# fishmarch/MS-SLAM

Measured on AMD Instinct MI355X. Metric: Mkeypoints/s extract+describe, KITTI-00-like stereo 1241x376, 2000 feat/frame, higher is better.
Workload: dtype u8

## Files before the change

### ms-slam_amd/csrc/gauss7_stream_device.h

```cpp
#pragma once
#include <hip/hip_runtime.h>
#include <stdint.h>

#include "orb_device.h"

namespace msorb {

typedef unsigned short ushort2v __attribute__((ext_vector_type(2)));

constexpr int kGaussRows = 28;
struct GaussTaps { uint32_t k[7]; };

struct BlurPlan {
    int block_begin[kMaxLevels + 1];
    int bx_count[kMaxLevels];
    int nlevels;
    uint32_t bx_magic[kMaxLevels];
    uint32_t image_magic;
};

__device__ __forceinline__ int refl101(int p, int len) { return p < 0 ? -p : (p >= len ? 2 * (len - 1) - p : p); }

constexpr int kGaussLanesOut = 62;
template <int ROWS, bool EDGE>
__device__ __forceinline__ void gauss7_strip(const uint8_t* __restrict__ sb, uint8_t* __restrict__ db, int src_pitch, int dst_pitch,
                                             int h, int y0, uint32_t xl, int x0, bool store, uint32_t sel_w1, uint32_t sel_w2a,
                                             uint32_t sel_w2b) {
    static_assert(ROWS % 28 == 0, "strips start on a multiple of 4 rows and the row loop is unrolled over 4 x 7 rows");
    uint8_t* const dblk = db + blur_tile_off((uint32_t)max(x0, 0), 0u, (uint32_t)dst_pitch);
    uint32_t blk[4] = {0u, 0u, 0u, 0u};
    auto load_row = [&](int r) {
        int yy = refl101(y0 - 3 + r, h);
        yy = min(max(yy, 0), h - 1);
        return *reinterpret_cast<const uint32_t*>(sb + (uint32_t)yy * (uint32_t)src_pitch + xl);
    };
    constexpr uint32_t k0 = 18, k1 = 34, k2 = 48, k3 = 56;
    constexpr uint32_t A0 = (k0 << 8) | (k1 << 16) | (k2 << 24), B0 = k3 | (k2 << 8) | (k1 << 16) | (k0 << 24);
    constexpr uint32_t A1 = (k0 << 16) | (k1 << 24), B1 = k2 | (k3 << 8) | (k2 << 16) | (k1 << 24), C1 = k0;
    constexpr uint32_t A2 = (k0 << 24), B2 = k1 | (k2 << 8) | (k3 << 16) | (k2 << 24), C2 = k1 | (k0 << 8);
    constexpr uint32_t B3 = k0 | (k1 << 8) | (k2 << 16) | (k3 << 24), C3 = k2 | (k1 << 8) | (k0 << 16);
    auto row_sums = [&](uint32_t w1, uint32_t hs[4]) {
        uint32_t w0 = (uint32_t)__builtin_amdgcn_update_dpp(0, (int)w1, 0x138 , 0xf, 0xf, true);
        uint32_t w2 = (uint32_t)__builtin_amdgcn_update_dpp(0, (int)w1, 0x130 , 0xf, 0xf, true);
        if (EDGE) {
            if (x0 == 0) w0 = __builtin_amdgcn_perm(0u, w1, 0x01020300u);
            const uint32_t n2 = __builtin_amdgcn_perm(w1, w0, sel_w2a) | __builtin_amdgcn_perm(0u, w2, sel_w2b);
            w1 = __builtin_amdgcn_perm(w1, w0, sel_w1);
            w2 = n2;
        }
        hs[0] = __builtin_amdgcn_udot4(w1, B0, __builtin_amdgcn_udot4(w0, A0, 0u, false), false);
        hs[1] = __builtin_amdgcn_udot4(w2, C1, __builtin_amdgcn_udot4(w1, B1, __builtin_amdgcn_udot4(w0, A1, 0u, false), false), false);
        hs[2] = __builtin_amdgcn_udot4(w2, C2, __builtin_amdgcn_udot4(w1, B2, __builtin_amdgcn_udot4(w0, A2, 0u, false), false), false);
        hs[3] = __builtin_amdgcn_udot4(w2, C3, __builtin_amdgcn_udot4(w1, B3, 0u, false), false);
    };
    const ushort2v K01 = {(unsigned short)k0, (unsigned short)k1}, K23 = {(unsigned short)k2, (unsigned short)k3},
                   K45 = {(unsigned short)k2, (unsigned short)k1};
    uint32_t acc[7][4];
    uint32_t hs[4], hp[4] = {0, 0, 0, 0};
    uint32_t warm[6], nxt[7];
#pragma unroll
    for (int r = 0; r < 6; r++) warm[r] = load_row(r);
#pragma unroll
    for (int u = 0; u < 7; u++) nxt[u] = load_row(6 + u);
#pragma unroll
    for (int r = 0; r < 6; r++) {
        row_sums(warm[r], hs);
#pragma unroll
        for (int j = 0; j < 4; j++) {
            if (r >= 1) {
                const ushort2v P = __builtin_bit_cast(ushort2v, hp[j] | (hs[j] << 16));
                acc[(r - 1) % 7][j] = __builtin_amdgcn_udot2(P, K01, 32768u, false);
                if (r >= 3) acc[(r - 3) % 7][j] = __builtin_amdgcn_udot2(P, K23, acc[(r - 3) % 7][j], false);
                if (r >= 5) acc[(r - 5) % 7][j] = __builtin_amdgcn_udot2(P, K45, acc[(r - 5) % 7][j], false);
            }
            hp[j] = hs[j];
        }
    }
#pragma unroll
    for (int it = 0; it < ROWS / 7; it++) {
        if (y0 + 7 * it >= h) break;
        uint32_t cur[7];
#pragma unroll
        for (int u = 0; u < 7; u++) cur[u] = nxt[u];
        if (it + 1 < ROWS / 7) {
#pragma unroll
            for (int u = 0; u < 7; u++) nxt[u] = load_row(6 + 7 * (it + 1) + u);
        }
#pragma unroll
        for (int u = 0; u < 7; u++) {
            const int r = 6 + 7 * it + u;
            row_sums(cur[u], hs);
            uint32_t q[4];
#pragma unroll
            for (int j = 0; j < 4; j++) {
                const ushort2v P = __builtin_bit_cast(ushort2v, hp[j] | (hs[j] << 16));
                q[j] = __umul24(hs[j], k0) + acc[u % 7][j];
                acc[(5 + u) % 7][j] = __builtin_amdgcn_udot2(P, K01, 32768u, false);
                acc[(3 + u) % 7][j] = __builtin_amdgcn_udot2(P, K23, acc[(3 + u) % 7][j], false);
                acc[(1 + u) % 7][j] = __builtin_amdgcn_udot2(P, K45, acc[(1 + u) % 7][j], false);
                hp[j] = hs[j];
            }
            const int o = r - 6;
            if (y0 + o < h) {
                const uint32_t packed = __builtin_amdgcn_perm(__builtin_amdgcn_perm(q[3], q[2], 0x0c0c0602u),
                                                              __builtin_amdgcn_perm(q[1], q[0], 0x0c0c0602u), 0x05040100u);
                blk[o & 3] = packed;
                if ((o & 3) == 3 || y0 + o == h - 1) {
                    if (store) *reinterpret_cast<uint4*>(dblk + (uint32_t)((y0 + o) >> 2) * ((uint32_t)dst_pitch * 4u)) = make_uint4(blk[0], blk[1], blk[2], blk[3]);
                }
            }
        }
    }
}

template <int ROWS>
__device__ __forceinline__ void gauss7_stream_body(const PyramidView& src, const PyramidView& dst, const BlurPlan& plan, const int tile, const int wave_in_block) {
    const int blocks_per_image = plan.block_begin[plan.nlevels];
    const int img = plan.image_magic ? (int)__umulhi((uint32_t)tile, plan.image_magic) : tile / blocks_per_image, blk = tile - img * blocks_per_image;
    int level = 0;
    while (level + 1 < plan.nlevels && blk >= plan.block_begin[level + 1]) level++;
    const int rem = blk - plan.block_begin[level];
    const int by = plan.bx_magic[level] ? (int)__umulhi((uint32_t)rem, plan.bx_magic[level]) : rem / plan.bx_count[level];
    const int bx = rem - by * plan.bx_count[level];
    const LevelView sv = src.lv[level], dv = dst.lv[level];
    const int lane = threadIdx.x & 63;
    const int x0 = (bx * kGaussLanesOut + lane - 1) * 4;
    const int y0 = (by * 4 + __builtin_amdgcn_readfirstlane(wave_in_block)) * ROWS;
    if (y0 >= sv.h) return;
    const bool store = lane >= 1 && (lane <= kGaussLanesOut || x0 + 4 >= sv.w) && x0 < sv.w;
    const bool border_block = (bx + 1) * kGaussLanesOut * 4 + 7 > sv.w;
    uint32_t sel_w1 = 0x07060504u, sel_w2a = 0x0c0c0c0cu, sel_w2b = 0x03020100u;
    if (border_block && x0 + 7 > sv.w && x0 < sv.w) {
        sel_w1 = 0; sel_w2a = 0; sel_w2b = 0;
        for (int b = 0; b < 8; b++) {
            const int x = x0 + b;
            int idx = b + 4;
            if (x >= sv.w) idx = max(2 * (sv.w - 1) - x, x0 - 4) - x0 + 4;
            if (b < 4) sel_w1 |= (uint32_t)idx << (8 * b);
            else {
                sel_w2a |= (uint32_t)(idx < 8 ? idx : 0x0c) << (8 * (b - 4));
                sel_w2b |= (uint32_t)(idx >= 8 ? idx - 8 : 0x0c) << (8 * (b - 4));
            }
        }
    }
    const uint32_t xl = (uint32_t)min(max(x0, 0), sv.pitch - 4);
    const uint8_t* sb = sv.base + (size_t)img * sv.img_stride;
    uint8_t* db = const_cast<uint8_t*>(dv.base) + (size_t)img * dv.img_stride;
    if (border_block || bx == 0)
        gauss7_strip<ROWS, true>(sb, db, sv.pitch, dv.pitch, sv.h, y0, xl, x0, store, sel_w1, sel_w2a, sel_w2b);
    else
        gauss7_strip<ROWS, false>(sb, db, sv.pitch, dv.pitch, sv.h, y0, xl, x0, store, sel_w1, sel_w2a, sel_w2b);
}

struct FrameBlurJob {
    PyramidView src, dst;
    BlurPlan plan;
    int blocks = 0;
};
bool make_frame_blur_job(const PyramidView& src, const PyramidView& dst, int n_images, const Semantics& sem, FrameBlurJob* job);

}
```

### ms-slam_amd/csrc/orb_kernels.hip

```cpp
#include <hip/hip_runtime.h>

#include <algorithm>
#include <string>
#include <stdint.h>
#include <stdlib.h>

#include "lds_limit.h"
#include "orb_device.h"
#include "gauss7_stream_device.h"
#include "sincosf_restated.h"

namespace msorb {

__global__ __launch_bounds__(256) void pyr_resize_kernel(LevelView src, LevelView dst, uint8_t* __restrict__ dst_base,
                                                         const ResizeTap* __restrict__ tx,
                                                         const ResizeTap* __restrict__ ty, int single_stage) {
    const int img = blockIdx.z;
    const int dy = blockIdx.y * 4 + (threadIdx.x >> 6);
    const int dx0 = (blockIdx.x * 64 + (threadIdx.x & 63)) * 4;
    if (dy >= dst.h || dx0 >= dst.w) return;
    const ResizeTap vy = ty[dy];
    const uint8_t* s0 = src.base + (size_t)img * src.img_stride + (size_t)vy.i0 * src.pitch;
    const uint8_t* s1 = src.base + (size_t)img * src.img_stride + (size_t)vy.i1 * src.pitch;
    const int b0 = vy.c0, b1 = vy.c1;
// ... 356 lines not shown
        colp_off = tr.colp;
        baseA = tr.rows_tbase >> 16;
    } else {
        int g_own, y_b;
        if (!by_wave) {
            const int strip = (int)(__umul24((uint32_t)tid, magic) >> 20);
            g_own = tid - strip * G;
            y_b = strip * R;
        } else {
            const int sl = (int)(__umul24((uint32_t)lane, magic) >> 20);
            g_own = lane - sl * G;
            const int y_w = (int)(((T == 128 ? cd.yw128 : cd.yw256) >> sw) & 255u);
            y_b = sl < (int)cd.spw ? y_w + sl * R : dh;
        }
        nrows = min(max(dh - y_b, 0), R);
        const int c_own = c_lo + 4 * g_own;
        const int xg = ga + c_own;
        const int vlo = min(max(x_lo - xg, 0), 4), vhi = min(max(x_hi - xg, 0), 4);
        Hm = (0x80808080u << (8 * vlo)) & (uint32_t)(0x0080808080ull >> (8 * (4 - vhi)));
        if (vlo >= 4) Hm = 0;
        colp_off = __umul24((uint32_t)y_b, P) + (uint32_t)c_own;
        baseA = (uint32_t)(((y_b + 3) << 7) | c_own);
    }
    tbase[tid] = (uint16_t)baseA;
    auto quick_test = [&](int th, uint32_t& wA, uint32_t& wB) {
        wA = 0; wB = 0;
        const uint8_t* colp = &tile[colp_off];
        uint32_t cw[GEO::kMaxR + 6], lw[GEO::kMaxR], rw_[GEO::kMaxR];
#pragma unroll
        for (int r = 0; r < GEO::kMaxR + 6; r++)
            if (r < 9 || r - 6 < R) cw[r] = *reinterpret_cast<const uint32_t*>(colp + r * P);
#pragma unroll
        for (int k = 0; k < GEO::kMaxR; k++)
            if (k < 3 || k < R) {
                lw[k] = *reinterpret_cast<const uint32_t*>(colp + (k + 3) * P - 4);
                rw_[k] = *reinterpret_cast<const uint32_t*>(colp + (k + 3) * P + 4);
            }
        const ushort2v t2 = __builtin_bit_cast(ushort2v, (uint32_t)th * 0x00010001u);
#pragma unroll
        for (int k = 0; k < GEO::kMaxR; k++) {
            if (k >= 3 && k >= R) break;
            const uint32_t V = cw[k + 3], U = cw[k], D = cw[k + 6];
            const uint32_t R3 = __builtin_amdgcn_alignbyte(rw_[k], V, 3);
            const uint32_t L3 = __builtin_amdgcn_alignbyte(V, lw[k], 1);
            const uint32_t Ve = V & 0x00ff00ffu, Vo = (V >> 8) & 0x00ff00ffu;
            const uint32_t Ae = __builtin_bit_cast(uint32_t, __builtin_elementwise_sub_sat(__builtin_bit_cast(ushort2v, Ve), t2));
            const uint32_t Ao = __builtin_bit_cast(uint32_t, __builtin_elementwise_sub_sat(__builtin_bit_cast(ushort2v, Vo), t2));
            const uint32_t Qd = ~(Ae | (Ao << 8));
            const uint32_t Be = __builtin_bit_cast(uint32_t, __builtin_elementwise_sub_sat(__builtin_bit_cast(ushort2v, Ve ^ 0x00ff00ffu), t2));
            const uint32_t Bo = __builtin_bit_cast(uint32_t, __builtin_elementwise_sub_sat(__builtin_bit_cast(ushort2v, Vo ^ 0x00ff00ffu), t2));
            const uint32_t Qb = Be | (Bo << 8);
            const uint32_t one = 0x01010101u;
            const uint32_t X = (__builtin_amdgcn_lerp(U, Qd, one) & __builtin_amdgcn_lerp(D, Qd, one)) |
                               (__builtin_amdgcn_lerp(L3, Qd, one) & __builtin_amdgcn_lerp(R3, Qd, one));
            const uint32_t Y = (__builtin_amdgcn_lerp(U, Qb, 0u) | __builtin_amdgcn_lerp(D, Qb, 0u)) &
                               (__builtin_amdgcn_lerp(L3, Qb, 0u) | __builtin_amdgcn_lerp(R3, Qb, 0u));
            const uint32_t hm = k < nrows ? Hm : 0u;
            const uint32_t z = (Y & hm) | ((~X & hm) >> 1);
            if (k < 4) wA |= z >> (6 - 2 * k);
            else wB |= z >> (6 - 2 * (k - 4));
        }
    };
    __syncthreads();

    const int sc_off = 4 - c_lo;
    Cand16* const out = slots + (size_t)img * slots_per_image + cd.slot_off;
    int n_emitted = 0;
    for (int pass = 0; pass < 2; pass++) {
        const int th = pass ? min_th : ini_th;
        uint32_t wA, wB;
        quick_test(th, wA, wB);
        const int cnt = __popc(wA) + __popc(wB);
        int n_work = 0;
        const int my_base = block_excl_scan<T / 64>(cnt, lane, wave, wave_tot[0], &n_work);

        const uint32_t baseB = baseA + (4u << 7);
        int w_begin = 0, n_corner = 0;
        if (n_work <= GEO::kWorkCap) {
            uint16_t* wp = &work[my_base];
            const uint32_t idA = (uint32_t)tid << 5, idB = idA | (1u << (5 + (T == 128 ? 7 : 8)));
            for (uint32_t w = wA; w; w &= w - 1) *wp++ = (uint16_t)(idA | (uint32_t)__builtin_ctz(w));
            for (uint32_t w = wB; w; w &= w - 1) *wp++ = (uint16_t)(idB | (uint32_t)__builtin_ctz(w));
            __syncthreads();
            w_begin = wave * ((((n_work + T / 64 - 1) / (T / 64)) + 63) & ~63);
            const int w_end = min(w_begin + ((((n_work + T / 64 - 1) / (T / 64)) + 63) & ~63), n_work);
            n_corner = 0;
            for (int i0 = w_begin; i0 < w_end; i0 += 64) {
                const int i = i0 + lane;
                bool corner = false;
                int ce = 0;
                if (i < w_end) {
                    const int id = work[i];
                    const int e = tbase[(id >> 5) & (T - 1)] + lut[id & 31] + ((id >> (5 + (T == 128 ? 7 : 8))) << 9);
                    const int ty = (e >> 7) & 127, tx = e & 127;
                    const int A = fast_arc_contrast_pk<GEO>(&tile[(int)__umul24((uint32_t)ty, P) + tx], (e & 0x8000) ? -1 : 1);
                    if (A > th) {
                        score[(int)__umul24((uint32_t)(ty - 2), SP) + tx + sc_off] = (uint8_t)(A - 1);
                        ce = e & 0x3FFF;
                        corner = true;
                    }
                }
                const unsigned long long bm = __ballot(corner);
                if (corner)
                    work[w_begin + n_corner + (int)__builtin_amdgcn_mbcnt_hi((uint32_t)(bm >> 32), __builtin_amdgcn_mbcnt_lo((uint32_t)bm, 0u))] = (uint16_t)ce;
                n_corner += __popcll(bm);
            }
        } else {
#pragma unroll 1
            for (int half = 0; half < 2; half++)
#pragma unroll 1
                for (uint32_t w = half ? wB : wA; w; w &= w - 1) {
                    const int e = lut[__builtin_ctz(w)] + (half ? baseB : baseA);
                    const int ty = (e >> 7) & 127, tx = e & 127;
                    const int A = fast_arc_contrast_pk<GEO>(&tile[(int)__umul24((uint32_t)ty, P) + tx], (e & 0x8000) ? -1 : 1);
                    if (A > th) score[(int)__umul24((uint32_t)(ty - 2), SP) + tx + sc_off] = (uint8_t)(A - 1);
                }
        }
        __syncthreads();

        if (n_work <= GEO::kWorkCap) {
            constexpr int wpr = GEO::kWordsPerRow;
            const int nwords = dh * wpr;
            uint32_t mine_keep = 0;
            {
                int slot = 0;
                for (int m0 = 0; m0 < n_corner; m0 += 64, slot++) {
                    if (m0 + lane >= n_corner) continue;
                    const int e = work[w_begin + m0 + lane];
                    const int ty = e >> 7, tx = e & 127;
                    const uint8_t* q = &score[(int)__umul24((uint32_t)(ty - 2), SP) + tx + sc_off];
                    const int sv = q[0];
                    int m = max3i(q[-SP - 1], q[-SP], q[-SP + 1]);
                    m = max3i(m, q[-1], q[1]);
                    m = max(m, max3i(q[SP - 1], q[SP], q[SP + 1]));
                    if (sv > m) {
                        const int bx = tx - c_lo, by = ty - 3;
                        const int b = by * (32 * wpr) + bx;
                        atomicOr(&kbits[b >> 5], 1u << (b & 31));
                        mine_keep |= 1u << slot;
                    }
                }
            }
            __syncthreads();
            const uint32_t myword = tid < nwords ? kbits[tid] : 0u;
            int n_out = 0;
            const int wprefix = block_excl_scan<T / 64>(__popc(myword), lane, wave, wave_tot[1], &n_out);
            if (tid < nwords) kprefix[tid] = wprefix;
            __syncthreads();
            {
                int slot = 0;
                for (int m0 = 0; m0 < n_corner; m0 += 64, slot++) {
                    if (!(mine_keep & (1u << slot))) continue;
                    const int e = work[w_begin + m0 + lane];
                    const int ty = e >> 7, tx = e & 127;
                    const int b = (ty - 3) * (32 * wpr) + (tx - c_lo);
                    const int rank = kprefix[b >> 5] + __popc(kbits[b >> 5] & ((1u << (b & 31)) - 1u));
                    Cand16 c;
                    c.x = (uint16_t)(ga + tx - kMinBorder);
                    c.y = (uint16_t)(cd.y0 + ty - kMinBorder);
                    c.score = score[(int)__umul24((uint32_t)(ty - 2), SP) + tx + sc_off];
                    c.pad = 0;
                    out[rank] = c;
                }
            }
            n_emitted = n_out;
        } else {
            const int n_task = dh * G;
            uint32_t tid_here = (uint32_t)tid;
            asm volatile("" : "+v"(tid_here));
            const int t_begin = (int)(__umul24(tid_here, (uint32_t)n_task) / T),
                      t_end = (int)(__umul24(tid_here + 1u, (uint32_t)n_task) / T);
            uint64_t keep = 0;
            {
                int y = (int)(__umul24((uint32_t)t_begin, magic) >> 20);
                int g = t_begin - y * G;
                for (int task = t_begin, k = 0; task < t_end; task++, k++) {
                    const uint8_t* sp = &score[(y + 1) * SP + 4 + 4 * g];
                    const uint32_t S = *reinterpret_cast<const uint32_t*>(sp);
                    if (S) {
#pragma unroll
                        for (int j = 0; j < 4; j++) {
                            const int sv = (S >> (8 * j)) & 255;
                            if (sv) {
                                const uint8_t* q = sp + j;
                                int m = max3i(q[-SP - 1], q[-SP], q[-SP + 1]);
                                m = max3i(m, q[-1], q[1]);
                                m = max(m, max3i(q[SP - 1], q[SP], q[SP + 1]));
                                if (sv > m) keep |= 1ull << (4 * k + j);
                            }
                        }
                    }
                    if (++g == G) { g = 0; y++; }
                }
            }
            int n_out = 0;
            int pos = block_excl_scan<T / 64>(__popcll(keep), lane, wave, wave_tot[1], &n_out);
            if (keep) {
                int y = (int)(__umul24((uint32_t)t_begin, magic) >> 20);
                int g = t_begin - y * G;
                uint64_t m = keep;
                for (int task = t_begin; task < t_end; task++, m >>= 4) {
                    uint32_t m4 = (uint32_t)m & 15u;
                    while (m4) {
                        const int j = __ffs(m4) - 1;
                        m4 &= m4 - 1;
                        Cand16 c;
                        c.x = (uint16_t)(gx0 + 4 * g + j - kMinBorder);
                        c.y = (uint16_t)(cd.y0 + 3 + y - kMinBorder);
                        c.score = score[(y + 1) * SP + 4 + 4 * g + j];
                        c.pad = 0;
                        out[pos++] = c;
                    }
                    if (++g == G) { g = 0; y++; }
                }
            }
            n_emitted = n_out;
        }
        if (n_emitted > 0 || pass == 1 || ini_th == min_th) break;
        __syncthreads();
        clear_planes();
        __syncthreads();
    }
    if (tid == 0) cell_count[(size_t)img * n_cells + cell_id] = n_emitted;
}

template <bool ALIGNED, class GEO>
__global__ __launch_bounds__(GEO::kThreads, GEO::kMinWaves) void fast_cells_kernel(PyramidView pyr, const CellDesc* __restrict__ cells,
                                                         const FastThreadRec* __restrict__ ttab,
                                                         int ini_th, int min_th, int slots_per_image,
                                                         Cand16* __restrict__ slots, int* __restrict__ cell_count,
                                                         int n_cells, uint32_t gx_magic) {
    fast_cells_body<ALIGNED, GEO>(pyr, cells, ttab, ini_th, min_th, slots_per_image, slots, cell_count, n_cells, gx_magic,
                                  blockIdx.y * gridDim.x + blockIdx.x, gridDim.x, gridDim.x * gridDim.y);
}

__global__ __launch_bounds__(256) void cand_scan_cells_kernel(const int* __restrict__ cell_count, int n_cells,
// ... 346 lines not shown
    return a;
}

__device__ __forceinline__ int wave_sum_dpp(int v) {
    v += __builtin_amdgcn_update_dpp(0, v, 0xB1 , 0xf, 0xf, false);
    v += __builtin_amdgcn_update_dpp(0, v, 0x4E , 0xf, 0xf, false);
    v += __builtin_amdgcn_update_dpp(0, v, 0x141 , 0xf, 0xf, false);
    v += __builtin_amdgcn_update_dpp(0, v, 0x140 , 0xf, 0xf, false);
    v += __builtin_amdgcn_update_dpp(0, v, 0x142 , 0xa, 0xf, false);
    v += __builtin_amdgcn_update_dpp(0, v, 0x143 , 0xc, 0xf, false);
    return __builtin_amdgcn_readlane(v, 63);
}

__device__ __forceinline__ int wave_sum8_fold(const int (&v)[8], int lane) {
    int w[4], x[2];
#pragma unroll
    for (int j = 0; j < 4; j++) {
        const auto r = __builtin_amdgcn_permlane32_swap((unsigned)v[j], (unsigned)v[j + 4], false, false);
        w[j] = (int)(r[0] + r[1]);
    }
    const bool b3 = (lane & 8) != 0, b2 = (lane & 4) != 0;
#pragma unroll
    for (int j = 0; j < 2; j++) {
        const int keep = b3 ? w[2 * j + 1] : w[2 * j], send = b3 ? w[2 * j] : w[2 * j + 1];
        x[j] = keep + __builtin_amdgcn_update_dpp(0, send, 0x140 , 0xf, 0xf, false);
    }
    const int keep = b2 ? x[1] : x[0], send = b2 ? x[0] : x[1];
    int s = keep + __builtin_amdgcn_update_dpp(0, send, 0x141 , 0xf, 0xf, false);
    s += __builtin_amdgcn_update_dpp(0, s, 0xB1 , 0xf, 0xf, false);
    s += __builtin_amdgcn_update_dpp(0, s, 0x4E , 0xf, 0xf, false);
    return s;
}

__device__ __forceinline__ int rint_small(float x) { return __float_as_int(__fadd_rn(x, 12582912.0f)) - 0x4B400000; }

constexpr int kBlkSlot = 1600;
typedef uint32_t u32x4u __attribute__((ext_vector_type(4), aligned(4)));
typedef float f32x2 __attribute__((ext_vector_type(2)));
constexpr int kKpPerWave = 4;
#ifndef MSORB_DESC_RAW_DEPTH
#define MSORB_DESC_RAW_DEPTH 4
#endif

__device__ __forceinline__ void glds16(const uint8_t* sbase, uint32_t voff, uint32_t lds_dst) {
    unsigned keep;
    asm volatile("s_mov_b32 %0, m0\n\ts_mov_b32 m0, %3\n\ts_nop 0\n\tglobal_load_lds_dwordx4 %1, %2\n\ts_mov_b32 m0, %0"
                 : "=&s"(keep)
                 : "v"(voff), "s"(sbase), "s"(lds_dst)
                 : "memory");
}
__device__ __forceinline__ void glds_wait_all() { asm volatile("s_waitcnt vmcnt(0)" ::: "memory"); }

constexpr unsigned long long kRoundMagic = 0x4B4000004B400000ull;
__device__ __forceinline__ f32x2 pk_add_bcast(f32x2 v, unsigned long long s) {
    f32x2 r; asm("v_pk_add_f32 %0, %1, %2 op_sel_hi:[1,0]" : "=v"(r) : "v"(v), "s"(s)); return r;
}
__device__ __forceinline__ uint32_t mad24s(uint32_t a, uint32_t s, uint32_t c) {
    uint32_t r; asm("v_mad_u32_u24 %0, %1, %2, %3" : "=v"(r) : "v"(a), "s"(s), "v"(c)); return r;
}

constexpr int kDescWaves = 4;
template <int kTap>
__global__ __launch_bounds__(64 * kDescWaves) __attribute__((amdgpu_waves_per_eu(6, 6))) void describe_kernel(PyramidView pyr, PyramidView blur, const SelRec* __restrict__ sel,
                                                       const int* __restrict__ sel_count, int sel_stride,
                                                       LevelScale scales, msorb_keypoint* __restrict__ kps,
                                                       uint8_t* __restrict__ desc, int out_stride, int atan2_fma, uint32_t gx_magic) {
    __shared__ __attribute__((aligned(16))) uint8_t patch[kDescWaves * kKpPerWave][kBlkSlot];
    __shared__ int mom[kDescWaves][16];
    __shared__ __attribute__((aligned(16))) float tri[kDescWaves * kKpPerWave][4];
    static_assert(sizeof(mom) + sizeof(tri) <= 1024, "six descriptor workgroups per CU");
    int img = blockIdx.y, bx = blockIdx.x;
    if ((gridDim.y & 7u) == 0) {
        const unsigned lin = blockIdx.y * gridDim.x + blockIdx.x;
        const unsigned xcd = lin & 7u, j = lin >> 3;
        const unsigned q = gx_magic ? __umulhi(j, gx_magic) : j / gridDim.x;
        img = (int)(q * 8 + xcd);
        bx = (int)(j - q * gridDim.x);
    }
    const int lane = threadIdx.x & 63;
    const int wave = __builtin_amdgcn_readfirstlane((int)(threadIdx.x >> 6));
    const int k_first = (bx * kDescWaves + wave) * kKpPerWave;
    const int n_sel = sel_count[img];
    if (bx * (kDescWaves * kKpPerWave) >= n_sel) return;
    const int seg = lane % 3, row3 = lane / 3;
    uint32_t wu[2][4], vm[2][4];
    uint32_t rrow_c[2];
    int vrow[2];
    const uint32_t U0 = (uint32_t)(16 * seg + 1) * 0x01010101u + 0x03020100u;
#pragma unroll
    for (int t = 0; t < 2; t++) {
        const int row = lane < 63 ? 21 * t + row3 : 63;
        const bool valid = row < 31;
        const int dd = c_tab.umax[valid ? (row < 15 ? 15 - row : row - 15) : 0];
        const uint32_t above = (uint32_t)(0x7f - 16 - dd) * 0x01010101u;
        const uint32_t atlo = valid ? (uint32_t)(0x80 - 16 + dd) * 0x01010101u : 0u;
#pragma unroll
        for (int d = 0; d < 4; d++) {
            const uint32_t U = U0 + (uint32_t)d * 0x04040404u;
            const uint32_t in7 = (U + atlo) & ~(U + above) & 0x80808080u;
            const uint32_t m = in7 >> 7;
            wu[t][d] = U & (in7 | (in7 - m));
            vm[t][d] = m;
        }
        rrow_c[t] = (uint32_t)min(row, 30);
        vrow[t] = row - 15;
    }
    const uint32_t seg16 = 16u * (uint32_t)seg;
    uint32_t bbrow[2], bbcol16[2];
#pragma unroll
    for (int t = 0; t < 2; t++) {
        const int slot = lane + 64 * t;
        bbrow[t] = (uint32_t)min(slot / 10, 9);
        bbcol16[t] = (uint32_t)(slot % 10) * 16u;
    }
    f32x2 patx[4], paty[4];
#pragma unroll
    for (int w = 0; w < 4; w++) {
        const uint32_t pw = *reinterpret_cast<const uint32_t*>(&c_tab.pattern[(w * 64 + lane) * 4]);
        patx[w] = f32x2{(float)(int8_t)(pw & 255u), (float)(int8_t)((pw >> 16) & 255u)};
        paty[w] = f32x2{(float)(int8_t)((pw >> 8) & 255u), (float)(int8_t)(pw >> 24)};
    }
    const float factor_pi = (float)(3.1415926535897932384626433832795 / 180.0);

    const SelRec* recs = sel + (size_t)img * sel_stride;
    SelRec R[kKpPerWave];
    uint32_t rl[3];
    static_assert(sizeof(SelRec) == sizeof(rl), "a selection record is three dwords");
    {
        const uint32_t* mine = reinterpret_cast<const uint32_t*>(recs + min(k_first + (lane & (kKpPerWave - 1)), n_sel - 1));
        for (int i = 0; i < 3; i++) rl[i] = mine[i];
#pragma unroll
        for (int kk = 0; kk < kKpPerWave; kk++) {
            uint32_t w[3];
            for (int i = 0; i < 3; i++) w[i] = __builtin_amdgcn_readlane(rl[i], kk);
            memcpy(&R[kk], w, sizeof(w));
        }
    }
    uint8_t* const lp0 = patch[wave * kKpPerWave];
    const uint32_t lds0 = __builtin_amdgcn_readfirstlane((uint32_t)(uintptr_t)(__attribute__((address_space(3))) uint8_t*)lp0);
    int RQ[kKpPerWave];
#pragma unroll
    for (int kk = 0; kk < kKpPerWave; kk++) {
        const SelRec& r = R[kk];
        const LevelView bv = blur.lv[r.level];
        RQ[kk] = ((18 + ((r.y - 18) & 3)) << 8) | (18 + ((r.x - 18) & 3));
        const uint8_t* bbase = bv.base + (size_t)img * bv.img_stride + (size_t)((r.y - 18) >> 2) * ((size_t)bv.pitch * 4) +
                               (size_t)((r.x - 18) >> 2) * 16;
        const uint32_t pitch4 = (uint32_t)bv.pitch * 4u;
        const uint32_t dst = lds0 + (uint32_t)kk * kBlkSlot;
        glds16(bbase, __umul24(bbrow[0], pitch4) + bbcol16[0], dst);
        if (lane < 100 - 64) glds16(bbase, __umul24(bbrow[1], pitch4) + bbcol16[1], dst + 1024u);
    }
    struct Raw { u32x4u rp[2]; uint32_t rsh[2]; };
    auto issue_raw = [&](const SelRec& r, Raw& L) {
        const LevelView lv = pyr.lv[r.level];
        const uint8_t* rrow = lv.base + (size_t)img * lv.img_stride + (size_t)(r.y - 15) * lv.pitch + (r.x - 15) - 4;
        const uint32_t rlow = (uint32_t)reinterpret_cast<uintptr_t>(rrow);
#pragma unroll
        for (int t = 0; t < 2; t++) {
            const uint32_t o = __umul24(rrow_c[t], (uint32_t)lv.pitch);
            L.rsh[t] = (rlow + o) & 3u;
            if (t == 0 ? lane < 63 : lane < 3 * (31 - 21))
                L.rp[t] = *reinterpret_cast<const u32x4u*>(rrow + (size_t)(o + seg16 + 4u - L.rsh[t]));
        }
    };
    Raw Lq[kKpPerWave];
#pragma unroll
    for (int kk = 0; kk < MSORB_DESC_RAW_DEPTH && kk < kKpPerWave; kk++) issue_raw(R[kk], Lq[kk]);
    int mv[2 * kKpPerWave];
#pragma unroll
    for (int kk = 0; kk < kKpPerWave; kk++) {
        if (kk + MSORB_DESC_RAW_DEPTH < kKpPerWave) issue_raw(R[kk + MSORB_DESC_RAW_DEPTH], Lq[kk + MSORB_DESC_RAW_DEPTH]);
        const Raw& L = Lq[kk];
        int m10 = 0, m01 = 0;
#pragma unroll
        for (int t = 0; t < 2; t++) {
            const u32x4u v = L.rp[t];
            const uint32_t nx = (uint32_t)__builtin_amdgcn_update_dpp(0, (int)v.x, 0x130 , 0xf, 0xf, false);
            const uint32_t sh = L.rsh[t];
            const uint32_t px0 = __builtin_amdgcn_alignbyte(v.y, v.x, sh), px1 = __builtin_amdgcn_alignbyte(v.z, v.y, sh);
            const uint32_t px2 = __builtin_amdgcn_alignbyte(v.w, v.z, sh), px3 = __builtin_amdgcn_alignbyte(nx, v.w, sh);
            uint32_t sI = __builtin_amdgcn_udot4(px0, vm[t][0], 0u, false);
            sI = __builtin_amdgcn_udot4(px1, vm[t][1], sI, false);
            sI = __builtin_amdgcn_udot4(px2, vm[t][2], sI, false);
            sI = __builtin_amdgcn_udot4(px3, vm[t][3], sI, false);
            uint32_t su = __builtin_amdgcn_udot4(px0, wu[t][0], 0u, false);
            su = __builtin_amdgcn_udot4(px1, wu[t][1], su, false);
            su = __builtin_amdgcn_udot4(px2, wu[t][2], su, false);
            su = __builtin_amdgcn_udot4(px3, wu[t][3], su, false);
            m10 += (int)su - 16 * (int)sI;
            m01 += vrow[t] * (int)sI;
        }
        mv[kk] = m10;
        mv[kKpPerWave + kk] = m01;
    }
    static_assert(kKpPerWave == 4, "wave_sum8_fold sums eight values");
    mom[wave][lane >> 2] = wave_sum8_fold(mv, lane);
    __syncthreads();
    if (wave == 0) {
        const int kp = lane & (kDescWaves * kKpPerWave - 1), wv = kp / kKpPerWave, kk = kp % kKpPerWave;
        const int q = 2 * (kk & 1) + (kk >> 1);
        const int m10v = mom[wv][q] + mom[wv][q + 4], m01v = mom[wv][q + 8] + mom[wv][q + 12];
        const float angle_v = fast_atan2_deg((float)m01v, (float)m10v, atan2_fma);
        float a_v, b_v;
        glibc_sincosf<true>(__fmul_rn(angle_v, factor_pi), &b_v, &a_v);
        if (lane < kDescWaves * kKpPerWave) *reinterpret_cast<float4*>(tri[lane]) = float4{angle_v, a_v, b_v, 0.f};
    }
    __syncthreads();
    glds_wait_all();
    if (k_first >= n_sel) return;
    __builtin_amdgcn_fence(__ATOMIC_ACQ_REL, "wavefront");
    __builtin_amdgcn_wave_barrier();
#pragma unroll
    for (int kk = 0; kk < kKpPerWave; kk++) {
        const SelRec r = R[kk];
        const float4 t4 = *reinterpret_cast<const float4*>(tri[wave * kKpPerWave + kk]);
        const float a = __int_as_float(__builtin_amdgcn_readfirstlane(__float_as_int(t4.y)));
        const float b = __int_as_float(__builtin_amdgcn_readfirstlane(__float_as_int(t4.z)));
        static_assert((kKpPerWave * kBlkSlot) % 16 == 0, "a wave's slots must start on a multiple of 16 bytes for the base to ride in qq");
        const uint8_t* bc = &patch[0][0] + kk * kBlkSlot;
        const int r_bias = 0x4B400000 - (RQ[kk] >> 8), q_bias = 0x4B400000 - (RQ[kk] & 255) - wave * (kKpPerWave * kBlkSlot / 4);
        const f32x2 a2 = {a, a}, b2 = {b, b}, nb2 = {-b, -b};
        unsigned long long word[4];
#pragma unroll
        for (int w = 0; w < 4; w++) {
            f32x2 rv, qv;
            if (kTap == 1) {
                rv = __builtin_elementwise_fma(paty[w], a2, patx[w] * b2);
                qv = __builtin_elementwise_fma(paty[w], nb2, patx[w] * a2);
            } else if (kTap == 2) {
                rv = patx[w] * b2 + paty[w] * a2;
                qv = patx[w] * a2 + paty[w] * nb2;
            } else {
                rv = __builtin_elementwise_fma(patx[w], b2, paty[w] * a2);
                qv = __builtin_elementwise_fma(patx[w], a2, paty[w] * nb2);
            }
            const f32x2 rf = pk_add_bcast(rv, kRoundMagic);
            const f32x2 qf = pk_add_bcast(qv, kRoundMagic);
            int tv[2];
#pragma unroll
            for (int j = 0; j < 2; j++) {
                const uint32_t rr = (uint32_t)(__float_as_int(rf[j]) - r_bias), qq = (uint32_t)(__float_as_int(qf[j]) - q_bias);
                const uint32_t off = (rr << 2) + mad24s(rr >> 2, 144u, mad24s(qq >> 2, 12u, qq));
                tv[j] = bc[off];
            }
            word[w] = __ballot(tv[0] < tv[1]);
        }
        if (k_first + kk >= n_sel) break;
        if (lane < 4) {
            unsigned long long* d = reinterpret_cast<unsigned long long*>(desc + ((size_t)img * out_stride + r.dst) * 32);
            d[lane] = lane == 0 ? word[0] : lane == 1 ? word[1] : lane == 2 ? word[2] : word[3];
        }
    }
    if (lane < kKpPerWave && k_first + lane < n_sel) {
        SelRec r;
        memcpy(&r, rl, sizeof(r));
        msorb_keypoint kp;
        const float sc = scales.scale[r.level];
        kp.x = r.level ? __fmul_rn((float)r.x, sc) : (float)r.x;
        kp.y = r.level ? __fmul_rn((float)r.y, sc) : (float)r.y;
        kp.size = scales.patch[r.level];
        kp.angle = tri[wave * kKpPerWave + lane][0];
        kp.response = (float)r.score;
        kp.octave = r.level;
        kp.class_id = -1;
        kps[(size_t)img * out_stride + r.dst] = kp;
    }
}

__global__ __launch_bounds__(256) void stage_level0_kernel(const uint8_t* __restrict__ src, size_t row_stride, size_t image_stride,
                                                           uint8_t* __restrict__ dst, int dst_pitch, size_t dst_image_stride,
                                                           int cols) {
    const int g = blockIdx.x * 256 + threadIdx.x;
    const int x = 4 * g;
    if (x >= cols) return;
// ... 413 lines not shown
```

Before: 497.8.

## Retile gauss strips, use buffer loads, interleave FAST work chunks, remap moment lanes

Doubles the Gaussian blur strip height to 56 rows, with a non-unrolled outer loop over 28-row groups, and loads source rows through a buffer resource using a wave-uniform row offset. In FAST, per-wave work chunks become interleaved across waves with a fixed stride instead of contiguous ranges. The orientation moment computation maps each lane to half a row (two lanes per row, 20 bytes each), so one load pass per keypoint replaces two. The goal is fewer redundant halo rows, less address arithmetic and fewer memory transactions, at the cost of fewer blur waves and changed load balance.

```diff
diff --git a/ms-slam_amd/csrc/gauss7_stream_device.h b/ms-slam_amd/csrc/gauss7_stream_device.h
--- a/ms-slam_amd/csrc/gauss7_stream_device.h
+++ b/ms-slam_amd/csrc/gauss7_stream_device.h
@@ -8,7 +8,10 @@
 
 typedef unsigned short ushort2v __attribute__((ext_vector_type(2)));
 
-constexpr int kGaussRows = 28;
+#ifndef MSORB_GAUSS_ROWS
+#define MSORB_GAUSS_ROWS 56
+#endif
+constexpr int kGaussRows = MSORB_GAUSS_ROWS;
 struct GaussTaps { uint32_t k[7]; };
 
 struct BlurPlan {
@@ -26,13 +29,14 @@
 __device__ __forceinline__ void gauss7_strip(const uint8_t* __restrict__ sb, uint8_t* __restrict__ db, int src_pitch, int dst_pitch,
                                              int h, int y0, uint32_t xl, int x0, bool store, uint32_t sel_w1, uint32_t sel_w2a,
                                              uint32_t sel_w2b) {
-    static_assert(ROWS % 28 == 0, "strips start on a multiple of 4 rows and the row loop is unrolled over 4 x 7 rows");
+    static_assert(ROWS % 28 == 0, "strips start on a multiple of 4 rows and the row loop's body is 4 x 7 rows");
     uint8_t* const dblk = db + blur_tile_off((uint32_t)max(x0, 0), 0u, (uint32_t)dst_pitch);
     uint32_t blk[4] = {0u, 0u, 0u, 0u};
+    const auto rsrc = __builtin_amdgcn_make_buffer_rsrc(const_cast<uint8_t*>(sb), 0, (int)((uint32_t)h * (uint32_t)src_pitch), 0x00020000);
     auto load_row = [&](int r) {
         int yy = refl101(y0 - 3 + r, h);
-        yy = min(max(yy, 0), h - 1);
-        return *reinterpret_cast<const uint32_t*>(sb + (uint32_t)yy * (uint32_t)src_pitch + xl);
+        yy = __builtin_amdgcn_readfirstlane(min(max(yy, 0), h - 1));
+        return (uint32_t)__builtin_amdgcn_raw_buffer_load_b32(rsrc, (int)xl, (int)((uint32_t)yy * (uint32_t)src_pitch), 0);
     };
     constexpr uint32_t k0 = 18, k1 = 34, k2 = 48, k3 = 56;
     constexpr uint32_t A0 = (k0 << 8) | (k1 << 16) | (k2 << 24), B0 = k3 | (k2 << 8) | (k1 << 16) | (k0 << 24);
@@ -76,37 +80,41 @@
             hp[j] = hs[j];
         }
     }
+    bool live = true;
+#pragma unroll 1
+    for (int g = 0; g < ROWS / 28 && live; g++) {
+        const int yg = y0 + 28 * g;
 #pragma unroll
-    for (int it = 0; it < ROWS / 7; it++) {
-        if (y0 + 7 * it >= h) break;
-        uint32_t cur[7];
+        for (int s = 0; s < 4; s++) {
+            if (yg + 7 * s >= h) { live = false; break; }
+            uint32_t cur[7];
 #pragma unroll
-        for (int u = 0; u < 7; u++) cur[u] = nxt[u];
-        if (it + 1 < ROWS / 7) {
+            for (int u = 0; u < 7; u++) cur[u] = nxt[u];
+            if (s < 3 || g + 1 < ROWS / 28) {
 #pragma unroll
-            for (int u = 0; u < 7; u++) nxt[u] = load_row(6 + 7 * (it + 1) + u);
-        }
+                for (int u = 0; u < 7; u++) nxt[u] = load_row(6 + 28 * g + 7 * (s + 1) + u);
+            }
 #pragma unroll
-        for (int u = 0; u < 7; u++) {
-            const int r = 6 + 7 * it + u;
-            row_sums(cur[u], hs);
-            uint32_t q[4];
+            for (int u = 0; u < 7; u++) {
+                row_sums(cur[u], hs);
+                uint32_t q[4];
 #pragma unroll
-            for (int j = 0; j < 4; j++) {
-                const ushort2v P = __builtin_bit_cast(ushort2v, hp[j] | (hs[j] << 16));
-                q[j] = __umul24(hs[j], k0) + acc[u % 7][j];
-                acc[(5 + u) % 7][j] = __builtin_amdgcn_udot2(P, K01, 32768u, false);
-                acc[(3 + u) % 7][j] = __builtin_amdgcn_udot2(P, K23, acc[(3 + u) % 7][j], false);
-                acc[(1 + u) % 7][j] = __builtin_amdgcn_udot2(P, K45, acc[(1 + u) % 7][j], false);
-                hp[j] = hs[j];
-            }
-            const int o = r - 6;
-            if (y0 + o < h) {
-                const uint32_t packed = __builtin_amdgcn_perm(__builtin_amdgcn_perm(q[3], q[2], 0x0c0c0602u),
-                                                              __builtin_amdgcn_perm(q[1], q[0], 0x0c0c0602u), 0x05040100u);
-                blk[o & 3] = packed;
-                if ((o & 3) == 3 || y0 + o == h - 1) {
-                    if (store) *reinterpret_cast<uint4*>(dblk + (uint32_t)((y0 + o) >> 2) * ((uint32_t)dst_pitch * 4u)) = make_uint4(blk[0], blk[1], blk[2], blk[3]);
+                for (int j = 0; j < 4; j++) {
+                    const ushort2v P = __builtin_bit_cast(ushort2v, hp[j] | (hs[j] << 16));
+                    q[j] = __umul24(hs[j], k0) + acc[u % 7][j];
+                    acc[(5 + u) % 7][j] = __builtin_amdgcn_udot2(P, K01, 32768u, false);
+                    acc[(3 + u) % 7][j] = __builtin_amdgcn_udot2(P, K23, acc[(3 + u) % 7][j], false);
+                    acc[(1 + u) % 7][j] = __builtin_amdgcn_udot2(P, K45, acc[(1 + u) % 7][j], false);
+                    hp[j] = hs[j];
+                }
+                const int ob = 7 * s + u, yo = yg + ob;
+                if (yo < h) {
+                    const uint32_t packed = __builtin_amdgcn_perm(__builtin_amdgcn_perm(q[3], q[2], 0x0c0c0602u),
+                                                                  __builtin_amdgcn_perm(q[1], q[0], 0x0c0c0602u), 0x05040100u);
+                    blk[ob & 3] = packed;
+                    if ((ob & 3) == 3 || yo == h - 1) {
+                        if (store) *reinterpret_cast<uint4*>(dblk + (uint32_t)(yo >> 2) * ((uint32_t)dst_pitch * 4u)) = make_uint4(blk[0], blk[1], blk[2], blk[3]);
+                    }
                 }
             }
         }
@@ -114,7 +122,8 @@
 }
 
 template <int ROWS>
-__device__ __forceinline__ void gauss7_stream_body(const PyramidView& src, const PyramidView& dst, const BlurPlan& plan, const int tile, const int wave_in_block) {
+__device__ __forceinline__ void gauss7_stream_body(const PyramidView& src, const PyramidView& dst, const BlurPlan& plan, const int tile_of_wave, const int wave_in_block) {
+    const int tile = __builtin_amdgcn_readfirstlane(tile_of_wave);
     const int blocks_per_image = plan.block_begin[plan.nlevels];
     const int img = plan.image_magic ? (int)__umulhi((uint32_t)tile, plan.image_magic) : tile / blocks_per_image, blk = tile - img * blocks_per_image;
     int level = 0;
diff --git a/ms-slam_amd/csrc/orb_kernels.hip b/ms-slam_amd/csrc/orb_kernels.hip
--- a/ms-slam_amd/csrc/orb_kernels.hip
+++ b/ms-slam_amd/csrc/orb_kernels.hip
@@ -462,14 +462,14 @@
             for (uint32_t w = wA; w; w &= w - 1) *wp++ = (uint16_t)(idA | (uint32_t)__builtin_ctz(w));
             for (uint32_t w = wB; w; w &= w - 1) *wp++ = (uint16_t)(idB | (uint32_t)__builtin_ctz(w));
             __syncthreads();
-            w_begin = wave * ((((n_work + T / 64 - 1) / (T / 64)) + 63) & ~63);
-            const int w_end = min(w_begin + ((((n_work + T / 64 - 1) / (T / 64)) + 63) & ~63), n_work);
+            constexpr int kChunkStride = (T / 64) * 64;
+            w_begin = (sw >> 3) * 64;
             n_corner = 0;
-            for (int i0 = w_begin; i0 < w_end; i0 += 64) {
+            for (int i0 = w_begin; i0 < n_work; i0 += kChunkStride) {
                 const int i = i0 + lane;
                 bool corner = false;
                 int ce = 0;
-                if (i < w_end) {
+                if (i < n_work) {
                     const int id = work[i];
                     const int e = tbase[(id >> 5) & (T - 1)] + lut[id & 31] + ((id >> (5 + (T == 128 ? 7 : 8))) << 9);
                     const int ty = (e >> 7) & 127, tx = e & 127;
@@ -481,8 +481,10 @@
                     }
                 }
                 const unsigned long long bm = __ballot(corner);
-                if (corner)
-                    work[w_begin + n_corner + (int)__builtin_amdgcn_mbcnt_hi((uint32_t)(bm >> 32), __builtin_amdgcn_mbcnt_lo((uint32_t)bm, 0u))] = (uint16_t)ce;
+                if (corner) {
+                    const int m = n_corner + (int)__builtin_amdgcn_mbcnt_hi((uint32_t)(bm >> 32), __builtin_amdgcn_mbcnt_lo((uint32_t)bm, 0u));
+                    work[w_begin + (m >> 6) * kChunkStride + (m & 63)] = (uint16_t)ce;
+                }
                 n_corner += __popcll(bm);
             }
         } else {
@@ -506,7 +508,7 @@
                 int slot = 0;
                 for (int m0 = 0; m0 < n_corner; m0 += 64, slot++) {
                     if (m0 + lane >= n_corner) continue;
-                    const int e = work[w_begin + m0 + lane];
+                    const int e = work[w_begin + m0 * (T / 64) + lane];
                     const int ty = e >> 7, tx = e & 127;
                     const uint8_t* q = &score[(int)__umul24((uint32_t)(ty - 2), SP) + tx + sc_off];
                     const int sv = q[0];
@@ -531,7 +533,7 @@
                 int slot = 0;
                 for (int m0 = 0; m0 < n_corner; m0 += 64, slot++) {
                     if (!(mine_keep & (1u << slot))) continue;
-                    const int e = work[w_begin + m0 + lane];
+                    const int e = work[w_begin + m0 * (T / 64) + lane];
                     const int ty = e >> 7, tx = e & 127;
                     const int b = (ty - 3) * (32 * wpr) + (tx - c_lo);
                     const int rank = kprefix[b >> 5] + __popc(kbits[b >> 5] & ((1u << (b & 31)) - 1u));
@@ -1044,30 +1046,27 @@
     const int k_first = (bx * kDescWaves + wave) * kKpPerWave;
     const int n_sel = sel_count[img];
     if (bx * (kDescWaves * kKpPerWave) >= n_sel) return;
-    const int seg = lane % 3, row3 = lane / 3;
-    uint32_t wu[2][4], vm[2][4];
-    uint32_t rrow_c[2];
-    int vrow[2];
-    const uint32_t U0 = (uint32_t)(16 * seg + 1) * 0x01010101u + 0x03020100u;
-#pragma unroll
-    for (int t = 0; t < 2; t++) {
-        const int row = lane < 63 ? 21 * t + row3 : 63;
+    const int seg = lane & 1;
+    const int row = lane < 62 ? lane >> 1 : 63;
+    uint32_t wu[5], vm[5];
+    const uint32_t U0 = (uint32_t)(20 * seg + 1) * 0x01010101u + 0x03020100u;
+    {
         const bool valid = row < 31;
         const int dd = c_tab.umax[valid ? (row < 15 ? 15 - row : row - 15) : 0];
         const uint32_t above = (uint32_t)(0x7f - 16 - dd) * 0x01010101u;
         const uint32_t atlo = valid ? (uint32_t)(0x80 - 16 + dd) * 0x01010101u : 0u;
 #pragma unroll
-        for (int d = 0; d < 4; d++) {
+        for (int d = 0; d < 5; d++) {
             const uint32_t U = U0 + (uint32_t)d * 0x04040404u;
             const uint32_t in7 = (U + atlo) & ~(U + above) & 0x80808080u;
             const uint32_t m = in7 >> 7;
-            wu[t][d] = U & (in7 | (in7 - m));
-            vm[t][d] = m;
-        }
-        rrow_c[t] = (uint32_t)min(row, 30);
-        vrow[t] = row - 15;
-    }
-    const uint32_t seg16 = 16u * (uint32_t)seg;
+            wu[d] = U & (in7 | (in7 - m));
+            vm[d] = m;
+        }
+    }
+    const uint32_t rrow_c = (uint32_t)min(row, 30);
+    const int vrow = row - 15;
+    const uint32_t seg20 = 20u * (uint32_t)seg;
     uint32_t bbrow[2], bbcol16[2];
 #pragma unroll
     for (int t = 0; t < 2; t++) {
@@ -1113,17 +1112,18 @@
         glds16(bbase, __umul24(bbrow[0], pitch4) + bbcol16[0], dst);
         if (lane < 100 - 64) glds16(bbase, __umul24(bbrow[1], pitch4) + bbcol16[1], dst + 1024u);
     }
-    struct Raw { u32x4u rp[2]; uint32_t rsh[2]; };
+    struct Raw { u32x4u rp; uint32_t r4, rsh; };
     auto issue_raw = [&](const SelRec& r, Raw& L) {
         const LevelView lv = pyr.lv[r.level];
         const uint8_t* rrow = lv.base + (size_t)img * lv.img_stride + (size_t)(r.y - 15) * lv.pitch + (r.x - 15) - 4;
         const uint32_t rlow = (uint32_t)reinterpret_cast<uintptr_t>(rrow);
-#pragma unroll
-        for (int t = 0; t < 2; t++) {
-            const uint32_t o = __umul24(rrow_c[t], (uint32_t)lv.pitch);
-            L.rsh[t] = (rlow + o) & 3u;
-            if (t == 0 ? lane < 63 : lane < 3 * (31 - 21))
-                L.rp[t] = *reinterpret_cast<const u32x4u*>(rrow + (size_t)(o + seg16 + 4u - L.rsh[t]));
+        const uint32_t o = __umul24(rrow_c, (uint32_t)lv.pitch);
+        L.rsh = (rlow + o) & 3u;
+        L.r4 = 0u;
+        if (lane < 62) {
+            const uint8_t* p = rrow + (size_t)(o + seg20 + 4u - L.rsh);
+            L.rp = *reinterpret_cast<const u32x4u*>(p);
+            if (seg == 0) L.r4 = *reinterpret_cast<const uint32_t*>(p + 16);
         }
     };
     Raw Lq[kKpPerWave];
@@ -1134,25 +1134,23 @@
     for (int kk = 0; kk < kKpPerWave; kk++) {
         if (kk + MSORB_DESC_RAW_DEPTH < kKpPerWave) issue_raw(R[kk + MSORB_DESC_RAW_DEPTH], Lq[kk + MSORB_DESC_RAW_DEPTH]);
         const Raw& L = Lq[kk];
-        int m10 = 0, m01 = 0;
-#pragma unroll
-        for (int t = 0; t < 2; t++) {
-            const u32x4u v = L.rp[t];
-            const uint32_t nx = (uint32_t)__builtin_amdgcn_update_dpp(0, (int)v.x, 0x130 , 0xf, 0xf, false);
-            const uint32_t sh = L.rsh[t];
-            const uint32_t px0 = __builtin_amdgcn_alignbyte(v.y, v.x, sh), px1 = __builtin_amdgcn_alignbyte(v.z, v.y, sh);
-            const uint32_t px2 = __builtin_amdgcn_alignbyte(v.w, v.z, sh), px3 = __builtin_amdgcn_alignbyte(nx, v.w, sh);
-            uint32_t sI = __builtin_amdgcn_udot4(px0, vm[t][0], 0u, false);
-            sI = __builtin_amdgcn_udot4(px1, vm[t][1], sI, false);
-            sI = __builtin_amdgcn_udot4(px2, vm[t][2], sI, false);
-            sI = __builtin_amdgcn_udot4(px3, vm[t][3], sI, false);
-            uint32_t su = __builtin_amdgcn_udot4(px0, wu[t][0], 0u, false);
-            su = __builtin_amdgcn_udot4(px1, wu[t][1], su, false);
-            su = __builtin_amdgcn_udot4(px2, wu[t][2], su, false);
-            su = __builtin_amdgcn_udot4(px3, wu[t][3], su, false);
-            m10 += (int)su - 16 * (int)sI;
-            m01 += vrow[t] * (int)sI;
-        }
+        const u32x4u v = L.rp;
+        const uint32_t nx = (uint32_t)__builtin_amdgcn_update_dpp(0, (int)v.x, 0x130 , 0xf, 0xf, false);
+        const uint32_t sh = L.rsh;
+        const uint32_t px0 = __builtin_amdgcn_alignbyte(v.y, v.x, sh), px1 = __builtin_amdgcn_alignbyte(v.z, v.y, sh);
+        const uint32_t px2 = __builtin_amdgcn_alignbyte(v.w, v.z, sh), px3 = __builtin_amdgcn_alignbyte(L.r4, v.w, sh);
+        const uint32_t px4 = __builtin_amdgcn_alignbyte(nx, L.r4, sh);
+        uint32_t sI = __builtin_amdgcn_udot4(px0, vm[0], 0u, false);
+        sI = __builtin_amdgcn_udot4(px1, vm[1], sI, false);
+        sI = __builtin_amdgcn_udot4(px2, vm[2], sI, false);
+        sI = __builtin_amdgcn_udot4(px3, vm[3], sI, false);
+        sI = __builtin_amdgcn_udot4(px4, vm[4], sI, false);
+        uint32_t su = __builtin_amdgcn_udot4(px0, wu[0], 0u, false);
+        su = __builtin_amdgcn_udot4(px1, wu[1], su, false);
+        su = __builtin_amdgcn_udot4(px2, wu[2], su, false);
+        su = __builtin_amdgcn_udot4(px3, wu[3], su, false);
+        su = __builtin_amdgcn_udot4(px4, wu[4], su, false);
+        const int m10 = (int)su - 16 * (int)sI, m01 = vrow * (int)sI;
         mv[kk] = m10;
         mv[kKpPerWave + kk] = m01;
     }
```

Result: slower. 487.4 (-2.1%).
